# PhilippBongartz/RepeatResolver

Hardware: AMD Instinct MI355X
Metric: sum-of-pairs DP cells/sec (higher is better)
Workload: dtype u32

## Files before the change

repeatresolver_amd/csrc/pwr_device.hip:

```cpp
#include <hip/hip_runtime.h>

#include <algorithm>
#include <chrono>
#include <cstdint>
#include <cstdio>
#include <cstdlib>
#include <cstring>
#include <new>
#include <thread>
#include <type_traits>
#include <vector>

#include "pwr.h"

#define PWR_INF 0x40000000u
#define PWR_BIG 0x7fffffff

struct Hdr {
    int W;
    int nslots;
    int nfree;
    int cur;
    int status;
    int stop;
// ... 967 lines not shown
            const int rel0 = y0 + lc - a;
            int tg[C];
            int run = PWR_BIG;
#pragma unroll
            for (int i = 0; i < C; ++i) {
                const int pm1 = i ? (int)Mprev[i > 0 ? i - 1 : 0] : pm1_0;
                const int d = pm1 + ldsS[wave][cs][sxc][lc + i];
                const int u = (int)Mprev[i] + ug[i];
                accC[i] = (accC[i] << 1) | ((d <= u) ? 1u : 0u);
                const int t3 = min(min(d, u), ig[i]);
                tg[i] = ((unsigned)(rel0 + i) < (unsigned)Bx) ? t3 : PWR_BIG;
                run = min(run, tg[i]);
            }
            const int incl = wave_incl_min(run);
            const int excl = __builtin_amdgcn_update_dpp(PWR_BIG, incl, DPP_WAVE_SHR1, 0xF, 0xF, false);
            const int P_end = min(P_in, __builtin_amdgcn_readlane(incl, 63));
            int p = min(P_in, excl);
            if (x != L - 1) {
#pragma unroll
                for (int i = 0; i < C; ++i) {
                    accA[i] = (accA[i] << 1) | ((tg[i] >= p) ? 1u : 0u);
                    p = min(p, tg[i]);
                    Mprev[i] = (rel0 + i < 0) ? PWR_INF : (unsigned)(gg[i] + p);
                }
            } else {
                unsigned Mn[C];
                unsigned fa = 0;
#pragma unroll
                for (int i = 0; i < C; ++i) {
                    fa |= (tg[i] >= p) ? (1u << i) : 0u;
                    p = min(p, tg[i]);
                    Mn[i] = (rel0 + i < 0) ? PWR_INF : (unsigned)(gg[i] + p);
                }
                const unsigned mrow = needP ? ePy : PWR_INF;
                const unsigned left0 = (unsigned)__builtin_amdgcn_update_dpp((int)mrow, (int)Mn[C - 1], DPP_WAVE_SHR1, 0xF, 0xF, false);
#pragma unroll
                for (int i = 0; i < C; ++i) {
                    const unsigned lf = i ? Mn[i > 0 ? i - 1 : 0] : left0;
                    const bool inb = (unsigned)(rel0 + i) < (unsigned)Bx;
                    accA[i] = (accA[i] << 1) | ((((fa >> i) & 1u) || (inb && Mn[i] == lf)) ? 1u : 0u);
                    lastM[wave * MS + lc + i] = inb ? Mn[i] : 0xffffffffu;
                    Mprev[i] = Mn[i];
                }
            }
            nacc = (x & 15) + 1;
            if (lane == 63) {
                ST64(MBP(wave, x), P_end, x + 1);
                ST64(MBM(wave, x), Mprev[C - 1], x + 1);
                if (ms == ms_hi) ST64(PTB(x), P_end, x + 1);
            }
            ran_prev = 1;
            V2_NEXT_ROW()
        }
        if (lane == 0) __hip_atomic_store(&rdone[wave], round + 1, __ATOMIC_RELAXED, __HIP_MEMORY_SCOPE_WORKGROUP);
        __syncthreads();
        if (UNI(__hip_atomic_load(&s_done, __ATOMIC_RELAXED, __HIP_MEMORY_SCOPE_WORKGROUP)) >= NW) break;
    }
    if (round >= max_rounds) {
        if (tid == 0) { m->ok = 0; atomicCAS(&st.hdr->status, 0, PWR_ERR_INTERNAL); }
        return;
    }
    if (tid == 0) {
        m->clk = (unsigned)(__builtin_amdgcn_s_memtime() - t_clk0);
        m->rclk = (unsigned)(__builtin_amdgcn_s_memrealtime() - t_real0);
        m->rounds = round;
        atomicAdd(&st.hdr->cells_computed, m->cells);
    }
#undef MBP
#undef MBM
#undef PTB
#undef LD64
#undef LD32LO
#undef ST64
}

#ifndef PWR_INTERIOR_CLS
#define PWR_INTERIOR_CLS 0
#endif
#define V3_TICKS() ((unsigned)(__builtin_amdgcn_s_memtime() >> 10))
#define V3_TIMEOUT_TICKS (1u << 19)
#define V4_RB 128

#ifdef PWR_DIAG
#define DG_DECL unsigned long long dg_wait_fast = 0, dg_wait_gen = 0, dg_wait_setup = 0, dg_t = 0, dg_t2 = 0, dg_cyc_int = 0, dg_cyc_gen16 = 0, dg_ts1 = 0, dg_ts2 = 0, dg_tl2 = 0; unsigned dg_log = 0; unsigned dg_int = 0, dg_gen16 = 0, dg_general = 0, dg_nowork = 0, dg_runs = 0, dg_switch = 0;
#define DG_T0() dg_t = __builtin_amdgcn_s_memtime();
#define DG_ADD(ACC) ACC += __builtin_amdgcn_s_memtime() - dg_t;
#define DG_INC(CNT, N) CNT += (N);
#define DG_T2() dg_t2 = __builtin_amdgcn_s_memtime();
#define DG_ADD2(ACC) ACC += __builtin_amdgcn_s_memtime() - dg_t2;
#else
#define DG_T2()
#define DG_ADD2(ACC)
#define DG_DECL
#define DG_T0()
#define DG_ADD(ACC)
#define DG_INC(CNT, N)
#endif
template <int NW, int C, bool WG1>
__global__ __launch_bounds__(WG1 ? NW * 64 : 128) void k_fill_v3(DState st, JobBufs jb)
{
    constexpr int MS = 64 * C, RS = NW * MS;
    constexpr int NL = WG1 ? NW : 1;
    constexpr int RB = WG1 ? 64 : V4_RB;
    __shared__ __attribute__((aligned(16))) int ldsS1[NL][2][4][MS];
    __shared__ unsigned long long rP[NL][RB], rM[NL][RB];
    __shared__ int wprog[NL], wdone;
    const int vjob = WG1 ? (int)blockIdx.x : (int)(blockIdx.x + 8 * blockIdx.z), lane = threadIdx.x & 63;
    const int role = WG1 ? 0 : UNI((int)threadIdx.x >> 6);
    const int wave = WG1 ? UNI((int)threadIdx.x >> 6) : (int)blockIdx.y;
    const int lw = WG1 ? wave : 0, wr = WG1 ? (wave + 1) % NW : 0;
    if (vjob >= jb.njobs_launched * jb.smax) return;
    const int job = vjob / jb.smax;
    const SegDesc *const sd = jb.seg + (size_t)job * SEG_MAX + (vjob % jb.smax);
    JobMeta *m = &jb.meta[job];
    if (st.hdr->fallback > 0 && jb.v2_follows) return;
    if (!m->active || m->L <= 0 || !m->ok || m->wide || !sd->active || NOT_MINE(jb, job)) return;
    const int seg_xb = UNI(sd->xb), seg_fin = UNI(sd->fin);
    const int L = UNI(sd->xe) - seg_xb;
    const int Lf = seg_fin ? L - 1 : L;
    const int x_own = UNI(sd->xown) - seg_xb;
    const int g_own = x_own >> 4;
    const int chkA = x_own > 0 ? x_own : -1, chkB = seg_fin ? -1 : L;
    unsigned *const chk_w = jb.chk + (((size_t)job * (SEG_MAX + 1) + sd->s) * 2 + 0) * (size_t)jb.NC;
    unsigned *const chk_t = jb.chk + (((size_t)job * (SEG_MAX + 1) + sd->s + 1) * 2 + 1) * (size_t)jb.NC;
    const unsigned long long t_clk0 = __builtin_amdgcn_s_memtime(), t_real0 = __builtin_amdgcn_s_memrealtime();
    for (int i = threadIdx.x; i < NL * RB; i += blockDim.x) { (&rP[0][0])[i] = 0; (&rM[0][0])[i] = 0; }
    if (threadIdx.x < NL) wprog[threadIdx.x] = 0;
    if (threadIdx.x == 0) wdone = 0;
    __syncthreads();

    const int wl = (wave + NW - 1) % NW;
    const unsigned tagbase = jb.tagbase;
    const size_t gstride = (size_t)jb.gstride;
    unsigned long long *const gmy = jb.gmb + (((size_t)job * NW + wave) * gstride + (size_t)sd->grow0) * 2;
    const unsigned long long *const gleftw = jb.gmb + (((size_t)job * NW + wl) * gstride + (size_t)sd->grow0) * 2;
    const unsigned long long *const gjob = jb.gmb + ((size_t)job * NW * gstride + (size_t)sd->grow0) * 2;
#define PTOT_PTR(AP, BP, R) (gjob + (((size_t)((((AP) + (BP) - 1 - lo) / MS) % NW)) * gstride + (size_t)(R)) * 2)
    int *const abortf = &m->abort;
#define GLD(PTR) __hip_atomic_load((PTR), __ATOMIC_RELAXED, __HIP_MEMORY_SCOPE_AGENT)
#define GST(PTR, VAL, ROW) __hip_atomic_store((PTR), ((unsigned long long)(tagbase | (unsigned)((ROW) + 1)) << 32) | (unsigned)(VAL), __ATOMIC_RELAXED, __HIP_MEMORY_SCOPE_AGENT)
#define GST2(PTR, VAL, TAG) __hip_atomic_store((PTR), ((unsigned long long)(TAG) << 32) | (unsigned)(VAL), __ATOMIC_RELAXED, __HIP_MEMORY_SCOPE_AGENT)
#define TAGOF(W64) ((unsigned)((W64) >> 32))
#define LLD(REF) __hip_atomic_load(&(REF), __ATOMIC_RELAXED, __HIP_MEMORY_SCOPE_WORKGROUP)
#define LST(REF, V) __hip_atomic_store(&(REF), (V), __ATOMIC_RELAXED, __HIP_MEMORY_SCOPE_WORKGROUP)

    if (!WG1 && role == 1) {
        for (unsigned it = 0;; ++it) {
            if (UNI(LLD(wdone))) break;
            const int wx = UNI(LLD(wprog[lw]));
            const int r = wx - 1 + lane;
            const bool inr = r >= 0 && r < L;
            unsigned long long p = 0, q = 0;
            int ab = 0;
            if (inr) { p = GLD(gleftw + 2 * (size_t)r); q = GLD(gleftw + 2 * (size_t)r + 1); }
            if ((it & 15u) == 15u) ab = GLD(abortf);
            if (inr) {
                const unsigned tagr = tagbase | (unsigned)(r + 1);
                if (TAGOF(p) == tagr && TAGOF(q) == tagr) {
                    LST(rP[lw][r & (RB - 1)], p);
                    __hip_atomic_store(&rM[lw][r & (RB - 1)], q, __ATOMIC_RELEASE, __HIP_MEMORY_SCOPE_WORKGROUP);
                }
            }
            if (UNI(ab)) break;
        }
        return;
    }

    const int lo = UNI(m->lo), hi = UNI(m->hi), W = UNI(m->W), B = st.B, H = st.H;
    const int *way = jb.way + (size_t)job * jb.Lmax + seg_xb;
    const uint8_t *seq = st.seq + st.rowoff[UNI(m->k)] + seg_xb;
    const int4 *rec2 = jb.rec2 + (size_t)job * jb.colcap * 2;
    uint32_t *dirs = jb.dirs + (size_t)job * jb.dirstride + (size_t)(seg_xb >> 4) * RS;
    unsigned *lastM = jb.lastM + (size_t)job * jb.NC;
    const int lc = lane * C;
#define V4_LOADS(MSX, SLOT, AU, AG, AI, GL)                                                      \
    {                                                                                            \
        const int yq_ = lo + (MSX) * MS - 1;                                                     \
        GL = (yq_ >= lo && yq_ <= hi) ? UNI(rec2[2 * (yq_ - lo) + 1].y) : 0;                     \
        int4 p_[C];                                                                              \
        _Pragma("unroll") for (int i = 0; i < C; ++i) {                                          \
// ... 99 lines not shown
    while (x < L && !dead) {
        ran_prev = UNI(ran_prev); gacc = UNI(gacc); nacc = UNI(nacc); blk = UNI(blk); ms = UNI(ms); cs = UNI(cs); gleft = UNI(gleft);
        x = UNI(x);
#ifdef PWR_DIAG
        if (ran_prev && !dg_tl2) { dg_tl2 = __builtin_amdgcn_s_memrealtime(); if (lane == 0 && sd->s * NW + wave < 680) { tl[2] = dg_tl2; tl[5] = (unsigned long long)x; } }
#endif
        if ((ran_prev || first_pending) && x < Lf) {
            unsigned long long bOm = __builtin_amdgcn_ballot_w64((dcf & 1u) != 0);
            const bool first = UNI(first_pending) != 0;
            if (first || ((bOm >> (x & 63)) & 1ull)) {
                first_pending = 0;
                unsigned long long bPm = __builtin_amdgcn_ballot_w64((dcf & 2u) != 0);
                unsigned long long bMm = __builtin_amdgcn_ballot_w64((dcf & 4u) != 0);
                unsigned long long bTm = __builtin_amdgcn_ballot_w64((dcf & 8u) != 0);
                if (first) { bOm |= 1ull << (x & 63); bMm |= 1ull << (x & 63); }
                V4_EARLY_MASKS()
                int dcaf = (int)(dca & 0xffffffu), dcb = min(dcaf + B, W);
                unsigned dcs = min(dca >> 24, 3u) * (unsigned)(MS * 4);
                if ((x >> 4) != gacc) { V4_FLUSH() gacc = x >> 4; }
                V4_ALIGN_ACC(x & 15)
                if (lane == 0) LST(wprog[lw], x);
                unsigned mlast_v = 0;
                if (first) {
                    const unsigned tagp = tagbase | (unsigned)x;
                    const int yq = lo + ms * MS - 1;
                    const bool needM = yq >= a_prev && yq < a_prev + Bx_prev;
                    unsigned long long eT = 0, eM = 0;
                    DG_T0()
#ifdef PWR_DIAG
                    const unsigned long long ev_t0 = __builtin_amdgcn_s_memrealtime();
#endif
                    const unsigned t0 = V3_TICKS();
                    for (unsigned spin = 1;; ++spin) {
                        eT = GLD(PTOT_PTR(a_prev, Bx_prev, x - 1));
                        eM = LLD(rM[lw][(x - 1) & (RB - 1)]);
                        if (UNI(TAGOF(eT)) == tagp && (!needM || UNI(TAGOF(eM)) == tagp)) break;
                        if ((spin & 1023u) == 0 && (V3_TICKS() - t0 > V3_TIMEOUT_TICKS || UNI(GLD(abortf)))) { dead = true; break; }
                        __builtin_amdgcn_s_sleep(1);
                    }
                    DG_ADD(dg_wait_gen)
#ifdef PWR_DIAG
                    if (lane == 0 && dg_general < 36) {
                        unsigned long long *ev = jb.diag + ((size_t)job * 32 + wave) * 4096 + 16 + 3 * dg_general;
                        ev[0] = (unsigned long long)x; ev[1] = ev_t0; ev[2] = __builtin_amdgcn_s_memrealtime();
                    }
#endif
                    DG_INC(dg_general, 1)
                    if (dead) break;
                    const int eTx = (int)UNI((unsigned)eT);
#pragma unroll
                    for (int i = 0; i < C; ++i) Mprev[i] = (unsigned)eTx;
                    mlast_v = yq < a_prev ? PWR_INF - (unsigned)gleft : (needM ? UNI((unsigned)eM) : (unsigned)eTx);
                    ran_prev = 1;
                } else if ((bMm >> (x & 63)) & 1ull) {
                    const unsigned tagp = tagbase | (unsigned)x;
                    unsigned long long w_ = LLD(rM[lw][(x - 1) & (RB - 1)]);
                    if (UNI(TAGOF(w_)) != tagp) {
                        DG_T0()
                        const unsigned t0 = V3_TICKS();
                        for (unsigned spin = 1;; ++spin) {
                            w_ = LLD(rM[lw][(x - 1) & (RB - 1)]);
                            if (UNI(TAGOF(w_)) == tagp) break;
                            if ((spin & 1023u) == 0 && (V3_TICKS() - t0 > V3_TIMEOUT_TICKS || UNI(GLD(abortf)))) { dead = true; break; }
                            __builtin_amdgcn_s_sleep(1);
                        }
                        DG_ADD(dg_wait_setup)
                        if (dead) break;
                    }
                    mlast_v = (unsigned)w_;
                }
                int ycol[C];
#pragma unroll
                for (int i = 0; i < C; ++i) ycol[i] = lo + ms * MS + lc + i;
                const char *const stab = (const char *)&ldsS1[lw][cs][0][lc];
                int sgr[C];
                {
                    const int *const srow0 = (const int *)(stab + __builtin_amdgcn_readlane((int)dcs, x & 63));
#pragma unroll
                    for (int i = 0; i < C; ++i) sgr[i] = srow0[i];
                }
                int af_done = a_prev;
                int g_af = 0, g_be = 0, g_cs = 0, g_cp = -1;
                DG_INC(dg_runs, 1)
                while (true) {
                    const int r_beg = x & 15, g0 = x - r_beg, r0 = g0 & 63;
                    int nrun = __builtin_ctz(~((unsigned)(bOm >> (r0 + r_beg)) & 0xffffu) | (1u << (16 - r_beg)));
                    nrun = min(nrun, Lf - x);
                    if (nrun <= 0) break;
                    const unsigned nPm = (unsigned)(bPm >> r0) & 0xffffu, kMm = (unsigned)(bMm >> r0) & 0xffffu, eTm = (unsigned)(bTm >> r0) & 0xffffu;
                    const unsigned p0 = (nPm >> r_beg) & 1u, m0 = (kMm >> r_beg) & 1u, t0_ = (eTm >> r_beg) & 1u;
                    const unsigned diff = ((nPm ^ (0u - p0)) | (kMm ^ (0u - m0)) | ((p0 & m0) ? 0u : (eTm ^ (0u - t0_)))) & 0xffffu;
                    const int nsame = __builtin_ctz((diff >> r_beg) | 0x10000u);
                    const bool mixed16 = r_beg == 0 && nrun == 16 && nsame < 16;
                    const int r_e = mixed16 ? 16 : r_beg + min(nrun, nsame);
                    const unsigned et_here = (eTm >> r_beg) & ((1u << (r_e - r_beg)) - 1u);
                    const int cls = mixed16 ? 3 : ((p0 & m0) ? (et_here ? 1 : 0) : ((p0 | m0 | t0_) == 0u ? 2 : 3));
                    if (gacc < 0) gacc = x >> 4;
#ifdef PWR_DIAG
                    if (!dg_ts1 && x >= 1024) dg_ts1 = __builtin_amdgcn_s_memrealtime();
                    if (!dg_ts2 && x >= 2048) dg_ts2 = __builtin_amdgcn_s_memrealtime();
#endif
                    if (WG1) {
                        const int need = g0 + 16 - RB + 2;
                        if (need > 0 && UNI(LLD(wprog[wr])) < need) {
                            DG_T0()
                            const unsigned t0 = V3_TICKS();
                            for (unsigned spin = 1;; ++spin) {
                                if (UNI(LLD(wprog[wr])) >= need) break;
                                if ((spin & 1023u) == 0 && (V3_TICKS() - t0 > V3_TIMEOUT_TICKS || UNI(GLD(abortf)))) { dead = true; break; }
                                __builtin_amdgcn_s_sleep(1);
                            }
                            DG_ADD(dg_wait_setup)
                            if (dead) break;
                        }
                    }
                    unsigned long long *const gq0 = gmy + 2 * (size_t)g0;
                    const unsigned tag_g0 = tagbase | (unsigned)g0;
                    const unsigned long long *const ringM = &rM[lw][g0 & (RB - 1)], *const ringP = &rP[lw][g0 & (RB - 1)];
                    if (g0 != g_cp) {
                        const int src = 4 * min(r0 + lane, 63);
                        g_af = __builtin_amdgcn_ds_bpermute(src, dcaf);
                        g_be = __builtin_amdgcn_ds_bpermute(src, dcb);
                        g_cs = __builtin_amdgcn_ds_bpermute(src, (int)dcs);
                        g_cp = g0;
                    }
                    auto group_row = [&](const int r, auto cls_, auto bits_) __attribute__((always_inline)) {
                        constexpr int CLS = decltype(cls_)::value;
                        constexpr bool BITS = decltype(bits_)::value;
                        bool bP = CLS <= 1 || CLS == 4, bM = CLS <= 1 || CLS == 4;
                        if (CLS == 3) { bP = (nPm >> r) & 1u; bM = (kMm >> r) & 1u; }
                        int af = 0, bend = 0;
                        if (CLS >= 2) af = __builtin_amdgcn_readlane(g_af, r);
                        if (CLS == 1 || CLS == 3 || CLS == 4) bend = __builtin_amdgcn_readlane(g_be, r);
                        const int Mleft_v = bM ? (int)mlast_v : (int)PWR_INF - gleft;
                        const int pm1_0 = __builtin_amdgcn_update_dpp(Mleft_v, (int)Mprev[C - 1], DPP_WAVE_SHR1, 0xF, 0xF, false);
                        int tg[C];
                        int run = FBIG;
#pragma unroll
                        for (int i = 0; i < C; ++i) {
                            const int pm1 = i ? (int)Mprev[i > 0 ? i - 1 : 0] : pm1_0;
                            const int d = pm1 + sgr[i];
                            const int u = (int)Mprev[i] + ug[i];
                            if (BITS) accC[i] = acc_push(accC[i], __builtin_amdgcn_sicmp(d, u, ICMP_SLE));
                            const int t3 = min(min(d, u), ig[i]);
                            bool inb = true;
                            if (CLS == 1 || CLS == 4) inb = ycol[i] < bend;
                            if (CLS == 2) inb = ycol[i] >= af;
                            if (CLS == 3) inb = (unsigned)(ycol[i] - af) < (unsigned)(bend - af);
                            tg[i] = inb ? t3 : FBIG;
                            run = min(run, tg[i]);
                        }
                        unsigned long long fM = 0;
                        unsigned fP = 0;
                        if (CLS != 2) {
                            fM = LLD(ringM[r]);
                            __builtin_amdgcn_sched_barrier(0);
                            fP = __hip_atomic_load((const unsigned *)&ringP[r], __ATOMIC_RELAXED, __HIP_MEMORY_SCOPE_WORKGROUP);
                        }
                        __builtin_amdgcn_sched_barrier(0);
#define V4_SCAN_STEP(CTRL, RMASK) { const int t_ = __builtin_amdgcn_update_dpp(PWR_BIG, incl, CTRL, RMASK, 0xF, false); incl = min(incl, t_); }
#define V4_FENCE() __builtin_amdgcn_sched_barrier(0)
                        int incl = run;
                        V4_SCAN_STEP(DPP_ROW_SHR(1), 0xF) V4_FENCE();
                        const int soff = __builtin_amdgcn_readlane(g_cs, r + 1);
                        V4_FENCE(); V4_SCAN_STEP(DPP_ROW_SHR(2), 0xF) V4_FENCE();
                        const int *const srow = (const int *)(stab + soff);
                        V4_FENCE(); V4_SCAN_STEP(DPP_ROW_SHR(4), 0xF) V4_FENCE();
#pragma unroll
                        for (int i = 0; i < C; ++i) sgr[i] = srow[i];
                        V4_FENCE(); V4_SCAN_STEP(DPP_ROW_SHR(8), 0xF) V4_FENCE();
                        const unsigned tagx = tag_g0 + (unsigned)(r + 1);
                        V4_FENCE(); V4_SCAN_STEP(DPP_ROW_BCAST15, 0xA) V4_FENCE();
                        V4_FENCE(); V4_SCAN_STEP(DPP_ROW_BCAST31, 0xC) V4_FENCE();
#undef V4_SCAN_STEP
#undef V4_FENCE
                        if (bP && __builtin_expect(UNI(TAGOF(fM)) != tagx, 0)) {
                            DG_T0()
                            const unsigned t0 = V3_TICKS();
                            for (unsigned spin = 1; !dead; ++spin) {
                                fM = LLD(ringM[r]);
                                __builtin_amdgcn_sched_barrier(0);
                                fP = __hip_atomic_load((const unsigned *)&ringP[r], __ATOMIC_RELAXED, __HIP_MEMORY_SCOPE_WORKGROUP);
                                if (UNI(TAGOF(fM)) == tagx) break;
                                if ((spin & 1023u) == 0 && (V3_TICKS() - t0 > V3_TIMEOUT_TICKS || UNI(GLD(abortf)))) { dead = true; break; }
                                __builtin_amdgcn_s_sleep(1);
                            }
                            DG_ADD(dg_wait_fast)
                        }
                        const int P_in_v = bP ? (int)fP : PWR_BIG;
                        const int P_end_v = min(P_in_v, incl);
                        const int pq = min(P_in_v, FBIG);
                        int p = min(__builtin_amdgcn_update_dpp(pq, incl, DPP_WAVE_SHR1, 0xF, 0xF, false), pq);
#pragma unroll
                        for (int i = 0; i < C; ++i) {
                            if (BITS) accA[i] = acc_push(accA[i], __builtin_amdgcn_sicmp(tg[i], p, ICMP_SGE));
                            p = min(p, tg[i]);
                            Mprev[i] = (unsigned)(CLS == 0 ? p : min(p, ig[i]));
                        }
                        mlast_v = (unsigned)fM;
                        if (lane == 63) {
                            if (WG1) {
                                GST2(gq0 + 2 * r, P_end_v, tagx);
                                LST(rP[wr][(g0 + r) & (RB - 1)], ((unsigned long long)tagx << 32) | (unsigned)P_end_v);
                                LST(rM[wr][(g0 + r) & (RB - 1)], ((unsigned long long)tagx << 32) | (unsigned)Mprev[C - 1]);
                            } else {
                                typedef unsigned v4u_ __attribute__((ext_vector_type(4)));
                                v4u_ w4_; w4_.x = (unsigned)P_end_v; w4_.y = tagx; w4_.z = Mprev[C - 1]; w4_.w = tagx;
                                asm volatile("global_store_dwordx4 %0, %1, %2 sc1\n\ts_nop 1" :: "v"(16 * r), "v"(w4_), "s"(gq0) : "memory");
                            }
                        }
                    };
                    int r_end = r_e;
                    DG_T2()
                    using WithBits = std::integral_constant<bool, true>;
                    using NoBits = std::integral_constant<bool, false>;
                    const bool warmup = (x >> 4) < g_own;
                    if (warmup && r_beg == 0 && r_e == 16 && cls != 3) {
                        if (cls == 0) {
#pragma unroll
                            for (int r = 0; r < 16; ++r) group_row(r, std::integral_constant<int, PWR_INTERIOR_CLS>{}, NoBits{});
                            DG_INC(dg_int, 16)
                            DG_ADD2(dg_cyc_int)
                        } else if (cls == 1) {
#pragma unroll
                            for (int r = 0; r < 16; ++r) group_row(r, std::integral_constant<int, 1>{}, NoBits{});
                        } else {
#pragma unroll
                            for (int r = 0; r < 16; ++r) group_row(r, std::integral_constant<int, 2>{}, NoBits{});
                        }
                    } else if (cls == 0 && r_beg == 0 && r_e == 16) {
#pragma unroll
                        for (int r = 0; r < 16; ++r) group_row(r, std::integral_constant<int, PWR_INTERIOR_CLS>{}, WithBits{});
                        DG_INC(dg_int, 16)
                        DG_ADD2(dg_cyc_int)
                    } else if (cls == 1 && r_beg == 0 && r_e == 16) {
#pragma unroll
                        for (int r = 0; r < 16; ++r) group_row(r, std::integral_constant<int, 1>{}, WithBits{});
                    } else if (cls == 3 && r_beg == 0 && r_e == 16) {
#pragma unroll
                        for (int r = 0; r < 16; ++r) group_row(r, std::integral_constant<int, 3>{}, WithBits{});
                    } else if (cls == 2 && r_beg == 0 && r_e == 16) {
#pragma unroll
                        for (int r = 0; r < 16; ++r) group_row(r, std::integral_constant<int, 2>{}, WithBits{});
                    } else {
                        int r = r_beg;
                        for (; r < r_end && (r & 3) && !dead; ++r) group_row(r, std::integral_constant<int, 3>{}, WithBits{});
#define V4_BLOCKS(K) for (; r + 4 <= r_end && !dead; r += 4) { group_row(r, std::integral_constant<int, K>{}, WithBits{}); group_row(r + 1, std::integral_constant<int, K>{}, WithBits{}); \
                                                               group_row(r + 2, std::integral_constant<int, K>{}, WithBits{}); group_row(r + 3, std::integral_constant<int, K>{}, WithBits{}); }
                        if (cls == 0) V4_BLOCKS(0)
                        else if (cls == 1) V4_BLOCKS(1)
                        else if (cls == 2) V4_BLOCKS(2)
#undef V4_BLOCKS
                        for (; r < r_end && !dead; ++r) group_row(r, std::integral_constant<int, 3>{}, WithBits{});
                        r_end = r;
                    }
                    if (!(cls == 0 && r_beg == 0 && r_e == 16)) { DG_INC(dg_gen16, r_end - r_beg) DG_ADD2(dg_cyc_gen16) }
                    x = g0 + r_end;
#ifdef PWR_DIAG
                    if (lane == 0 && dg_log < 1270) {
                        unsigned long long *lg = jb.diag + ((size_t)job * 32 + wave) * 4096 + 256 + 3 * dg_log;
                        lg[0] = (unsigned long long)x | ((unsigned long long)cls << 32) | ((unsigned long long)(r_end - r_beg) << 40); lg[1] = __builtin_amdgcn_s_memrealtime();
                        lg[2] = dg_wait_fast + dg_wait_gen + dg_wait_setup;
                    }
                    dg_log += 1;
#endif
                    af_done = __builtin_amdgcn_readlane(dcaf, (x - 1) & 63);
                    if ((x & 15) == 0) {
                        uint32_t *d_ = dirs + (size_t)gacc * RS + (size_t)wave * MS + (size_t)lc;
#pragma unroll
                        for (int i = 0; i < C; ++i) { if (gacc >= g_own) d_[i] = accA[i] | (accC[i] << 16); accA[i] = accC[i] = 0; }
                        gacc = -1; nacc = 0;
                        V4_CHK_STORE(x, af_done, min(af_done + B, W))
                    } else nacc = x & 15;
                    if (dead || x >= Lf) break;
                    if ((x >> 6) != blk) {
                        V4_ROTATE_BLOCK()
                        bOm = __builtin_amdgcn_ballot_w64((dcf & 1u) != 0); bPm = __builtin_amdgcn_ballot_w64((dcf & 2u) != 0);
                        bMm = __builtin_amdgcn_ballot_w64((dcf & 4u) != 0); bTm = __builtin_amdgcn_ballot_w64((dcf & 8u) != 0);
                        V4_EARLY_MASKS()
                        dcaf = (int)(dca & 0xffffffu); dcb = min(dcaf + B, W);
                        dcs = min(dca >> 24, 3u) * (unsigned)(MS * 4);
                        g_cp = -1;
                        const int *const srow0 = (const int *)(stab + __builtin_amdgcn_readlane((int)dcs, 0));
#pragma unroll
                        for (int i = 0; i < C; ++i) sgr[i] = srow0[i];
                    }
                    if (lane == 0) LST(wprog[lw], x);
                }
                a_prev = af_done; Bx_prev = min(B, W - af_done);
                if (dead) break;
                if (x < L) {
                    if ((x >> 6) != blk) V4_ROTATE_BLOCK()
                    a = max(0, __builtin_amdgcn_readlane(wcur, x & 63) - H);
                    sx = __builtin_amdgcn_readlane(scur, x & 63);
                }
                if (lane == 0) LST(wprog[lw], x);
                continue;
            }
        }
        if (dead || x >= L) break;

        x = UNI(x); ms = UNI(ms); msn = UNI(msn); a = UNI(a); a_prev = UNI(a_prev); Bx_prev = UNI(Bx_prev);
        sx = UNI(sx); gacc = UNI(gacc); nacc = UNI(nacc); blk = UNI(blk); gleft = UNI(gleft); gleftn = UNI(gleftn); ran_prev = UNI(ran_prev); cs = UNI(cs);
        const int Bx = min(B, W - a);
        const int ms_lo = (a - lo) / MS, ms_hi = (a + Bx - 1 - lo) / MS;
        if (ms < ms_lo) {
            ms += NW;
            if (ms == msn) {
#pragma unroll
                for (int i = 0; i < C; ++i) { ug[i] = nu[i]; gg[i] = ng[i]; ig[i] = ni[i]; }
                gleft = gleftn;
                cs ^= 1;
            } else {
                while (ms < ms_lo) ms += NW;
                V4_LOADS(ms, cs, ug, gg, ig, gleft)
            }
            DG_INC(dg_switch, 1)
            msn = ms + NW;
            V4_LOADS(msn, cs ^ 1, nu, ng, ni, gleftn)
            ran_prev = 0;
            continue;
        }
        if (ms > ms_hi) {
            const int y0s = lo + ms * MS;
            const int anf_l = (int)(dca & 0xffffffu);
            const unsigned long long wm = __builtin_amdgcn_ballot_w64(min(anf_l + B, W) > y0s) >> (x & 63);
            const int xn = min(wm ? x + __builtin_ctzll(wm) : ((x >> 6) + 1) << 6, L);
            int xs = xn;
            if (wm && xn < Lf) {
                const int anf_up = __builtin_amdgcn_update_dpp(0x3fffffff, anf_l, DPP_WAVE_SHR1, 0xF, 0xF, false);
                const unsigned long long tears = __builtin_amdgcn_ballot_w64(anf_l >= min(anf_up + B, W)) >> (x & 63);
                const unsigned long long tm = tears & (~0ull >> (63 - (xn - x))) & ~1ull;
                xs = max(x, xn & ~15);
                if (tm) xs = max(xs, x + 63 - __builtin_clzll(tm));
                if (xs < 1) xs = xn;
                const int an = __builtin_amdgcn_readlane(anf_l, xn & 63);
                if (ms < (an - lo) / MS) { xs = xn; first_pending = 0; }
                else { early_lo = xs; early_hi = xn; first_pending = xs > 0 ? 1 : 0; }
            }
            DG_INC(dg_nowork, xs - x)
            if (xs > x) {
                const int al = __builtin_amdgcn_readlane((int)dca, (xs - 1) & 63) & 0xffffff;
                a_prev = al; Bx_prev = min(B, W - al);
            }
// ... 48 lines not shown
            DG_ADD(dg_wait_gen)
            DG_INC(dg_general, 1)
            if (dead) break;
        }
        int Mleft = (int)PWR_INF;
        if (x == 0) Mleft = (src_c < 0 || yq == src_c) ? -gleft : (int)PWR_INF - gleft;
        else if (yq < a_prev) Mleft = (int)PWR_INF - gleft;
        else if (needM) Mleft = (int)eMy;
        else Mleft = (int)eTx;
        const int P_in = needP ? (int)ePx : PWR_BIG;
        if (x > 0 && !ran_prev) {
#pragma unroll
            for (int i = 0; i < C; ++i) Mprev[i] = eTx;
        }
        if ((x >> 4) != gacc) { V4_FLUSH() gacc = x >> 4; }
        V4_ALIGN_ACC(x & 15)
        const int pm1_0 = __builtin_amdgcn_update_dpp(Mleft, (int)Mprev[C - 1], DPP_WAVE_SHR1, 0xF, 0xF, false);
        const int sxc = min(max(sx, 0), 3);
        const int rel0 = y0 + lc - a;
        int tg[C];
        int run = PWR_BIG;
#pragma unroll
        for (int i = 0; i < C; ++i) {
            const int pm1 = i ? (int)Mprev[i > 0 ? i - 1 : 0] : pm1_0;
            const int d = pm1 + ldsS1[lw][cs][sxc][lc + i];
            const int u = (int)Mprev[i] + ug[i];
            accC[i] = (accC[i] << 1) | ((d <= u) ? 1u : 0u);
            const int t3 = min(min(d, u), ig[i]);
            tg[i] = ((unsigned)(rel0 + i) < (unsigned)Bx) ? t3 : PWR_BIG;
            run = min(run, tg[i]);
        }
        const int incl = wave_incl_min(run);
        const int excl = __builtin_amdgcn_update_dpp(PWR_BIG, incl, DPP_WAVE_SHR1, 0xF, 0xF, false);
        const int P_end = min(P_in, __builtin_amdgcn_readlane(incl, 63));
        int p = min(P_in, excl);
        if (x != Lf) {
#pragma unroll
            for (int i = 0; i < C; ++i) {
                accA[i] = (accA[i] << 1) | ((tg[i] >= p) ? 1u : 0u);
                p = min(p, tg[i]);
                Mprev[i] = (unsigned)((rel0 + i < 0) ? ig[i] : p);
            }
        } else {
            unsigned Mn[C];
            unsigned fa = 0;
#pragma unroll
            for (int i = 0; i < C; ++i) {
                fa |= (tg[i] >= p) ? (1u << i) : 0u;
                p = min(p, tg[i]);
                Mn[i] = (rel0 + i < 0) ? PWR_INF : (unsigned)(gg[i] + p);
                Mprev[i] = (unsigned)((rel0 + i < 0) ? ig[i] : p);
            }
            const unsigned mrow = needP ? (unsigned)gleft + ePy : PWR_INF;
            const unsigned left0 = (unsigned)__builtin_amdgcn_update_dpp((int)mrow, (int)Mn[C - 1], DPP_WAVE_SHR1, 0xF, 0xF, false);
#pragma unroll
            for (int i = 0; i < C; ++i) {
                const unsigned lf = i ? Mn[i > 0 ? i - 1 : 0] : left0;
                const bool inb = (unsigned)(rel0 + i) < (unsigned)Bx;
                accA[i] = (accA[i] << 1) | ((((fa >> i) & 1u) || (inb && Mn[i] == lf)) ? 1u : 0u);
                lastM[wave * MS + lc + i] = inb ? Mn[i] : 0xffffffffu;
            }
        }
        nacc = (x & 15) + 1;
        if (lane == 63) {
            GST(gmy + 2 * (size_t)x, P_end, x);
            if (WG1) {
                const unsigned long long tg_ = (unsigned long long)(tagbase | (unsigned)(x + 1)) << 32;
                LST(rP[wr][x & (RB - 1)], tg_ | (unsigned)P_end);
                LST(rM[wr][x & (RB - 1)], tg_ | (unsigned)Mprev[C - 1]);
            } else GST(gmy + 2 * (size_t)x + 1, Mprev[C - 1], x);
        }
        ran_prev = 1;
        V4_CHK_STORE(x + 1, a, a + Bx)
        V4_NEXT_ROW()
    }
    V4_FLUSH()
#ifdef PWR_DIAG
    if (lane == 0) {
        unsigned long long *dgp = jb.diag + ((size_t)job * 32 + wave) * 4096;
        dgp[0] = __builtin_amdgcn_s_memtime() - t_clk0; dgp[1] = dg_wait_fast; dgp[2] = dg_wait_gen; dgp[3] = dg_wait_setup;
        dgp[4] = ((unsigned long long)dg_int << 32) | dg_gen16; dgp[5] = ((unsigned long long)dg_general << 32) | dg_nowork;
        dgp[6] = ((unsigned long long)dg_runs << 32) | dg_switch; dgp[7] = (unsigned long long)L;
        dgp[12] = dg_log; dgp[8] = dg_cyc_gen16; dgp[9] = dg_ts1; dgp[10] = dg_ts2; dgp[11] = dg_cyc_int;
    }
#endif
#ifdef PWR_DIAG
    if (lane == 0 && sd->s * NW + wave < 680) { tl[3] = __builtin_amdgcn_s_memrealtime(); tl[4] = (unsigned long long)L | ((unsigned long long)(dg_wait_fast + dg_wait_gen + dg_wait_setup) << 20); }
#endif
    if (lane == 0) { LST(wprog[lw], 0x7fffffff); LST(wdone, 1); }
    if (dead) {
        if (lane == 0) __hip_atomic_store(abortf, 1, __ATOMIC_RELAXED, __HIP_MEMORY_SCOPE_AGENT);
        return;
    }
    if (wave == 0 && lane == 0) {
        if (sd->s == 0) {
            m->clk = (unsigned)(__builtin_amdgcn_s_memtime() - t_clk0);
            m->rclk = (unsigned)(__builtin_amdgcn_s_memrealtime() - t_real0);
            m->rounds = 0;
        }
        atomicAdd(&st.hdr->cells_computed, sd->cells);
    }
#undef V4_CHK_STORE
#undef V4_EARLY_MASKS
#undef PTOT_PTR
#undef GLD
#undef GST
#undef GST2
#undef TAGOF
#undef LLD
#undef LST
#undef V4_LOADS
#undef V4_ALIGN_ACC
#undef V4_FLUSH
#undef V4_ROTATE_BLOCK
#undef V4_NEXT_ROW
}

__device__ __forceinline__ bool seg_check_applies(const DState &st, const JobBufs &jb, int job, const JobMeta *m)
{
    return m->active && m->L > 0 && m->ok && !m->wide && !m->abort && !(st.hdr->fallback > 0 && jb.v2_follows) && !NOT_MINE(jb, job) && m->nseg > 1;
}

__device__ __forceinline__ void seg_check_body(const DState &st, const JobBufs &jb, const int job, const int s, const int tid)
{
    __shared__ int s_min[4], s_max[4], s_bad;
    JobMeta *m = &jb.meta[job];
    if (!seg_check_applies(st, jb, job, m)) return;
    if (s >= m->nseg) return;
    const SegDesc *sd = jb.seg + (size_t)job * SEG_MAX + s;
    const int xr = sd->xown - 1;
    const int lo = m->lo, W = m->W, B = st.B, H = st.H, RS = jb.NC;
    const int a = max(0, jb.way[(size_t)job * jb.Lmax + xr] - H), Bx = min(B, W - a);
    unsigned *cw = jb.chk + (((size_t)job * (SEG_MAX + 1) + s) * 2 + 0) * (size_t)jb.NC;
    unsigned *ct = jb.chk + (((size_t)job * (SEG_MAX + 1) + s) * 2 + 1) * (size_t)jb.NC;
    if (tid == 0) s_bad = 0;
    __syncthreads();
    int dmin = INT_MAX, dmax = INT_MIN, bad = 0;
    for (int j = tid; j < Bx; j += 256) {
        const int idx = (a + j - lo) % RS;
        const unsigned vw = cw[idx], vt = ct[idx];
        if (vw == 0xffffffffu || vt == 0xffffffffu) bad = 1;
        else if ((vw >= PWR_INF) != (vt >= PWR_INF)) bad = 1;
        else if (vw < PWR_INF) { const int d = (int)(vw - vt); dmin = min(dmin, d); dmax = max(dmax, d); }
    }
    for (int o = 32; o > 0; o >>= 1) { dmin = min(dmin, __shfl_xor(dmin, o)); dmax = max(dmax, __shfl_xor(dmax, o)); }
    if ((tid & 63) == 0) { s_min[tid >> 6] = dmin; s_max[tid >> 6] = dmax; }
    if (bad) s_bad = 1;
    __syncthreads();
    for (int j = tid; j < RS; j += 256) { cw[j] = 0xffffffffu; ct[j] = 0xffffffffu; }
    if (tid == 0) {
        const int lo_ = min(min(s_min[0], s_min[1]), min(s_min[2], s_min[3])), hi_ = max(max(s_max[0], s_max[1]), max(s_max[2], s_max[3]));
        if (s_bad || (lo_ != INT_MAX && lo_ != hi_)) __hip_atomic_store(&m->segfail, 1, __ATOMIC_RELAXED, __HIP_MEMORY_SCOPE_AGENT);
        if (s == 1) { atomicAdd(&st.hdr->seg_jobs, 1ull); atomicAdd(&st.hdr->segs, (unsigned long long)m->nseg); }
        __hip_atomic_fetch_add(&jb.chkdone[job], 1, __ATOMIC_RELEASE, __HIP_MEMORY_SCOPE_AGENT);
    }
}

__global__ __launch_bounds__(256) void k_seg_check(DState st, JobBufs jb)
{
    seg_check_body(st, jb, (int)blockIdx.x, (int)blockIdx.y + 1, (int)threadIdx.x);
}

#define F64_NT 1024
#define F64_INF (1ll << 62)
__global__ __launch_bounds__(F64_NT) void k_fill64(DState st, JobBufs jb)
{
// ... 2771 lines not shown
    return PWR_OK;
}

extern "C" int pwr_reset_stats(pwr_ctx *c)
{
    if (!c) return PWR_ERR_ARG;
    if (c->on_device) {
        if (hipSetDevice(c->device) != hipSuccess) return PWR_ERR_DEVICE;
        int rc0 = drain_events(c);
        if (rc0) return rc0;
    }
    c->stats = pwr_stats{};
    if (c->on_device) {
        if (hipSetDevice(c->device) != hipSuccess) return PWR_ERR_DEVICE;
        HIPC(hipStreamSynchronize(c->stream));
        HIPC(hipMemset(&c->st.hdr->cells_computed, 0, 16 * sizeof(unsigned long long)));
        HIPC(hipMemset(&c->st.hdr->rows_jumped, 0, sizeof(unsigned long long)));
    }
    return PWR_OK;
}

extern "C" int pwr_debug_last_job(pwr_ctx *c, int *L, int *entry, int *W, int *way, int *newcol, int cap)
{
    if (!c || !c->on_device) return PWR_ERR_ARG;
    if (hipSetDevice(c->device) != hipSuccess) return PWR_ERR_DEVICE;
    HIPC(hipStreamSynchronize(c->stream));
    JobMeta m;
    HIPC(hipMemcpy(&m, c->jb.meta, sizeof m, hipMemcpyDeviceToHost));
    if (L) *L = m.L;
    if (entry) *entry = m.entry;
    if (W) *W = m.W;
    const int n = std::min(cap, m.L);
    if (way && n > 0) HIPC(hipMemcpy(way, c->jb.way, sizeof(int) * n, hipMemcpyDeviceToHost));
    if (newcol && n > 0) HIPC(hipMemcpy(newcol, c->jb.newcol, sizeof(int) * n, hipMemcpyDeviceToHost));
    return PWR_OK;
}

extern "C" int pwr_debug_row_columns(pwr_ctx *c, int k, int *out, int cap)
{
    if (!c || !c->on_device || k < 0 || k >= c->T || !out) return PWR_ERR_ARG;
    if (hipSetDevice(c->device) != hipSuccess) return PWR_ERR_DEVICE;
    const int L = c->rowlen[k];
    if (L == 0) return 0;
    int *d = nullptr;
    int rc = dmalloc(c, &d, (size_t)L);
    if (rc) return rc;
    hipLaunchKernelGGL(k_rowcols, dim3(32), dim3(256), 0, c->stream, c->st, k, d);
    std::vector<int> h(L);
    if (hipMemcpyAsync(h.data(), d, sizeof(int) * L, hipMemcpyDeviceToHost, c->stream) != hipSuccess || hipStreamSynchronize(c->stream) != hipSuccess) { dfree(c, d); return PWR_ERR_DEVICE; }
    dfree(c, d);
    memcpy(out, h.data(), sizeof(int) * std::min(L, cap));
    return L;
}

extern "C" int pwr_debug_rounds(pwr_ctx *c)
{
    if (!c || !c->on_device) return PWR_ERR_ARG;
    if (hipSetDevice(c->device) != hipSuccess) return PWR_ERR_DEVICE;
    if (hipStreamSynchronize(c->stream) != hipSuccess) return PWR_ERR_DEVICE;
    JobMeta m;
    if (hipMemcpy(&m, c->jb.meta, sizeof m, hipMemcpyDeviceToHost) != hipSuccess) return PWR_ERR_DEVICE;
    return m.rounds;
}

extern "C" int pwr_debug_phase_times(pwr_ctx *c, unsigned long long *out)
{
    if (!c || !c->on_device || !out) return PWR_ERR_ARG;
    if (hipSetDevice(c->device) != hipSuccess) return PWR_ERR_DEVICE;
    HIPC(hipStreamSynchronize(c->stream));
    HIPC(hipMemcpy(out, c->st.hdr->dbg, sizeof(unsigned long long) * 32, hipMemcpyDeviceToHost));
    HIPC(hipMemset(c->st.hdr->dbg, 0, sizeof(unsigned long long) * 32));
    return PWR_OK;
}

extern "C" int pwr_debug_fill_diag(pwr_ctx *c, unsigned long long *out)
{
    if (!c || !c->on_device || !out) return PWR_ERR_ARG;
    if (hipSetDevice(c->device) != hipSuccess) return PWR_ERR_DEVICE;
    HIPC(hipStreamSynchronize(c->stream));
    HIPC(hipMemcpy(out, c->jb.diag, sizeof(unsigned long long) * 32 * 4096, hipMemcpyDeviceToHost));
    return PWR_OK;
}

extern "C" int pwr_debug_fill_clock(pwr_ctx *c, double *mhz, double *fill_us)
{
    if (!c || !c->on_device) return PWR_ERR_ARG;
    if (hipSetDevice(c->device) != hipSuccess) return PWR_ERR_DEVICE;
    HIPC(hipStreamSynchronize(c->stream));
    JobMeta m;
    HIPC(hipMemcpy(&m, c->jb.meta, sizeof m, hipMemcpyDeviceToHost));
    if (mhz) *mhz = m.rclk ? 100.0 * (double)m.clk / (double)m.rclk : 0.0;
    if (fill_us) *fill_us = (double)m.rclk / 100.0;
    return PWR_OK;
}
```

Before: 54.95 billion.

## Merge consecutive same-class 16-row groups into multi-group runs

```diff
diff --git a/repeatresolver_amd/csrc/pwr_device.hip b/repeatresolver_amd/csrc/pwr_device.hip
--- a/repeatresolver_amd/csrc/pwr_device.hip
+++ b/repeatresolver_amd/csrc/pwr_device.hip
@@ -1073,20 +1073,73 @@
 #define V4_RB 128
 
 #ifdef PWR_DIAG
-#define DG_DECL unsigned long long dg_wait_fast = 0, dg_wait_gen = 0, dg_wait_setup = 0, dg_t = 0, dg_t2 = 0, dg_cyc_int = 0, dg_cyc_gen16 = 0, dg_ts1 = 0, dg_ts2 = 0, dg_tl2 = 0; unsigned dg_log = 0; unsigned dg_int = 0, dg_gen16 = 0, dg_general = 0, dg_nowork = 0, dg_runs = 0, dg_switch = 0;
+#define DG_DECL unsigned long long dg_wait_fast = 0, dg_wait_gen = 0, dg_wait_setup = 0, dg_t = 0, dg_t2 = 0, dg_cyc_int = 0, dg_cyc_gen16 = 0, dg_ts1 = 0, dg_ts2 = 0, dg_tl2 = 0; unsigned dg_log = 0; unsigned dg_int = 0, dg_gen16 = 0, dg_general = 0, dg_nowork = 0, dg_runs = 0, dg_switch = 0; \
+    unsigned long long dg_tg = 0, dg_glue = 0; unsigned dg_ngl = 0, dg_gcont = 0, dg_gother = 0; int dg_pkey = -1, dg_pend = -1;
 #define DG_T0() dg_t = __builtin_amdgcn_s_memtime();
 #define DG_ADD(ACC) ACC += __builtin_amdgcn_s_memtime() - dg_t;
 #define DG_INC(CNT, N) CNT += (N);
 #define DG_T2() dg_t2 = __builtin_amdgcn_s_memtime();
 #define DG_ADD2(ACC) ACC += __builtin_amdgcn_s_memtime() - dg_t2;
+#define DG_GLUE_RESET() dg_tg = 0;
+#define DG_GROUP_BEGIN(KEY, G0, WHOLE)                                                           \
+    {                                                                                            \
+        if (dg_tg) { dg_glue += __builtin_amdgcn_s_memtime() - dg_tg; dg_ngl += 1; }             \
+        if ((WHOLE) && dg_pkey == (int)(KEY) && dg_pend == (G0)) dg_gcont += 1; else dg_gother += 1;  \
+        dg_pkey = (WHOLE) ? (int)(KEY) : -1; dg_pend = (G0) + 16;                                \
+    }
+#define DG_GROUP_END() dg_tg = __builtin_amdgcn_s_memtime();
 #else
 #define DG_T2()
 #define DG_ADD2(ACC)
+#define DG_GLUE_RESET()
+#define DG_GROUP_BEGIN(KEY, G0, WHOLE)
+#define DG_GROUP_END()
 #define DG_DECL
 #define DG_T0()
 #define DG_ADD(ACC)
 #define DG_INC(CNT, N)
 #endif
+struct V4Run { int cls, r_e, ngrp; };
+__host__ __device__ static inline int v4_group_cls(const unsigned nPm, const unsigned kMm, const unsigned eTm)
+{
+    const unsigned p0 = nPm & 1u, m0 = kMm & 1u, t0_ = eTm & 1u;
+    const unsigned diff = ((nPm ^ (0u - p0)) | (kMm ^ (0u - m0)) | ((p0 & m0) ? 0u : (eTm ^ (0u - t0_)))) & 0xffffu;
+    if (diff) return 3;
+    return (p0 & m0) ? (eTm ? 1 : 0) : ((p0 | m0 | t0_) == 0u ? 2 : 3);
+}
+__host__ __device__ static inline V4Run v4_classify_run(const unsigned long long bOm, const unsigned long long bPm, const unsigned long long bMm,
+                                                        const unsigned long long bTm, const int x, const int g_own, const int Lf,
+                                                        const int early_lo, const int early_hi)
+{
+    V4Run out = {3, x & 15, 0};
+    const int r_beg = x & 15, g0 = x - r_beg, r0 = g0 & 63;
+    int nrun = __builtin_ctz(~((unsigned)(bOm >> (r0 + r_beg)) & 0xffffu) | (1u << (16 - r_beg)));
+    nrun = nrun < Lf - x ? nrun : Lf - x;
+    if (nrun <= 0) return out;
+    const unsigned nPm = (unsigned)(bPm >> r0) & 0xffffu, kMm = (unsigned)(bMm >> r0) & 0xffffu, eTm = (unsigned)(bTm >> r0) & 0xffffu;
+    out.ngrp = 1;
+    if (r_beg == 0 && nrun == 16) {
+        out.cls = v4_group_cls(nPm, kMm, eTm);
+        out.r_e = 16;
+        const bool warm = (g0 >> 4) < g_own;
+        if (early_hi >= g0 && early_lo < g0 + 16) return out;
+        for (int k = 1; r0 + 16 * k < 64; ++k) {
+            const int gk = g0 + 16 * k, rk = r0 + 16 * k;
+            if (gk + 16 > Lf || ((gk >> 4) < g_own) != warm || (early_hi >= gk && early_lo < gk + 16)) break;
+            if (((unsigned)(bOm >> rk) & 0xffffu) != 0xffffu) break;
+            if (v4_group_cls((unsigned)(bPm >> rk) & 0xffffu, (unsigned)(bMm >> rk) & 0xffffu, (unsigned)(bTm >> rk) & 0xffffu) != out.cls) break;
+            out.ngrp = k + 1;
+        }
+        return out;
+    }
+    const unsigned p0 = (nPm >> r_beg) & 1u, m0 = (kMm >> r_beg) & 1u, t0_ = (eTm >> r_beg) & 1u;
+    const unsigned diff = ((nPm ^ (0u - p0)) | (kMm ^ (0u - m0)) | ((p0 & m0) ? 0u : (eTm ^ (0u - t0_)))) & 0xffffu;
+    const int nsame = __builtin_ctz((diff >> r_beg) | 0x10000u);
+    out.r_e = r_beg + (nrun < nsame ? nrun : nsame);
+    const unsigned et_here = (eTm >> r_beg) & ((1u << (out.r_e - r_beg)) - 1u);
+    out.cls = (p0 & m0) ? (et_here ? 1 : 0) : ((p0 | m0 | t0_) == 0u ? 2 : 3);
+    return out;
+}
 template <int NW, int C, bool WG1>
 __global__ __launch_bounds__(WG1 ? NW * 64 : 128) void k_fill_v3(DState st, JobBufs jb)
 {
@@ -1352,19 +1405,17 @@
                 int af_done = a_prev;
                 int g_af = 0, g_be = 0, g_cs = 0, g_cp = -1;
                 DG_INC(dg_runs, 1)
+                DG_GLUE_RESET()
                 while (true) {
-                    const int r_beg = x & 15, g0 = x - r_beg, r0 = g0 & 63;
-                    int nrun = __builtin_ctz(~((unsigned)(bOm >> (r0 + r_beg)) & 0xffffu) | (1u << (16 - r_beg)));
-                    nrun = min(nrun, Lf - x);
-                    if (nrun <= 0) break;
-                    const unsigned nPm = (unsigned)(bPm >> r0) & 0xffffu, kMm = (unsigned)(bMm >> r0) & 0xffffu, eTm = (unsigned)(bTm >> r0) & 0xffffu;
-                    const unsigned p0 = (nPm >> r_beg) & 1u, m0 = (kMm >> r_beg) & 1u, t0_ = (eTm >> r_beg) & 1u;
-                    const unsigned diff = ((nPm ^ (0u - p0)) | (kMm ^ (0u - m0)) | ((p0 & m0) ? 0u : (eTm ^ (0u - t0_)))) & 0xffffu;
-                    const int nsame = __builtin_ctz((diff >> r_beg) | 0x10000u);
-                    const bool mixed16 = r_beg == 0 && nrun == 16 && nsame < 16;
-                    const int r_e = mixed16 ? 16 : r_beg + min(nrun, nsame);
-                    const unsigned et_here = (eTm >> r_beg) & ((1u << (r_e - r_beg)) - 1u);
-                    const int cls = mixed16 ? 3 : ((p0 & m0) ? (et_here ? 1 : 0) : ((p0 | m0 | t0_) == 0u ? 2 : 3));
+                    const int r_beg = x & 15;
+                    int g0 = x - r_beg, r0 = g0 & 63;
+                    const V4Run run = v4_classify_run(bOm, bPm, bMm, bTm, x, g_own, Lf, early_lo, early_hi);
+                    if (run.ngrp <= 0) break;
+                    unsigned nPm = (unsigned)(bPm >> r0) & 0xffffu, kMm = (unsigned)(bMm >> r0) & 0xffffu;
+                    const int r_e = run.r_e, cls = run.cls;
+#ifdef PWR_DIAG
+                    const int dg_x0 = x;
+#endif
                     if (gacc < 0) gacc = x >> 4;
 #ifdef PWR_DIAG
                     if (!dg_ts1 && x >= 1024) dg_ts1 = __builtin_amdgcn_s_memrealtime();
@@ -1384,9 +1435,9 @@
                             if (dead) break;
                         }
                     }
-                    unsigned long long *const gq0 = gmy + 2 * (size_t)g0;
-                    const unsigned tag_g0 = tagbase | (unsigned)g0;
-                    const unsigned long long *const ringM = &rM[lw][g0 & (RB - 1)], *const ringP = &rP[lw][g0 & (RB - 1)];
+                    unsigned long long *gq0 = gmy + 2 * (size_t)g0;
+                    unsigned tag_g0 = tagbase | (unsigned)g0;
+                    const unsigned long long *ringM = &rM[lw][g0 & (RB - 1)], *ringP = &rP[lw][g0 & (RB - 1)];
                     if (g0 != g_cp) {
                         const int src = 4 * min(r0 + lane, 63);
                         g_af = __builtin_amdgcn_ds_bpermute(src, dcaf);
@@ -1481,38 +1532,73 @@
                         }
                     };
                     int r_end = r_e;
-                    DG_T2()
                     using WithBits = std::integral_constant<bool, true>;
                     using NoBits = std::integral_constant<bool, false>;
                     const bool warmup = (x >> 4) < g_own;
+#define V4_RUN_NEXT(NAF, NBE, NCS)                                                               \
+                    {                                                                            \
+                        const int xg_ = g0 + 16;                                                 \
+                        if (xg_ == chkA || xg_ == chkB) break;        \
+                        uint32_t *d_ = dirs + (size_t)gacc * RS + (size_t)wave * MS + (size_t)lc; \
+                        _Pragma("unroll") for (int i = 0; i < C; ++i) { if (gacc >= g_own) d_[i] = accA[i] | (accC[i] << 16); accA[i] = accC[i] = 0; } \
+                        if (lane == 0) LST(wprog[lw], xg_);                                      \
+                        if (WG1) {                                                               \
+                            const int need_ = xg_ + 16 - RB + 2;                                 \
+                            if (need_ > 0 && UNI(LLD(wprog[wr])) < need_) {                      \
+                                DG_T0()                                                          \
+                                const unsigned t0_ = V3_TICKS();                                 \
+                                for (unsigned spin = 1;; ++spin) {                               \
+                                    if (UNI(LLD(wprog[wr])) >= need_) break;                     \
+                                    if ((spin & 1023u) == 0 && (V3_TICKS() - t0_ > V3_TIMEOUT_TICKS || UNI(GLD(abortf)))) { dead = true; break; } \
+                                    __builtin_amdgcn_s_sleep(1);                                 \
+                                }                                                                \
+                                DG_ADD(dg_wait_setup)                                            \
+                                if (dead) break;      \
+                            }                                                                    \
+                        }                                                                        \
+                        gacc += 1; g0 = xg_; r0 += 16;                                           \
+                        gq0 += 32; tag_g0 += 16u; ringM += 16; ringP += 16;                      \
+                        nPm = (unsigned)(bPm >> r0) & 0xffffu; kMm = (unsigned)(bMm >> r0) & 0xffffu; \
+                        g_af = NAF; g_be = NBE; g_cs = NCS; g_cp = g0;                           \
+                    }
+#ifdef PWR_DIAG
+#define V4_RUN_DIAG_BEGIN() { if (!dg_ts1 && g0 >= 1024) dg_ts1 = __builtin_amdgcn_s_memrealtime(); if (!dg_ts2 && g0 >= 2048) dg_ts2 = __builtin_amdgcn_s_memrealtime(); } \
+                        DG_GROUP_BEGIN(cls | (warmup ? 8 : 0) | ((g0 >> 6) << 4), g0, true) DG_T2()
+#define V4_RUN_DIAG_END() if (cls == 0) { DG_INC(dg_int, 16) DG_ADD2(dg_cyc_int) } else { DG_INC(dg_gen16, 16) DG_ADD2(dg_cyc_gen16) } DG_GROUP_END()
+#else
+#define V4_RUN_DIAG_BEGIN()
+#define V4_RUN_DIAG_END()
+#endif
+#define V4_RUN(CLSK, BITS)                                                                       \
+                    for (int gi = run.ngrp;; --gi) {                                             \
+                        int n_af = 0, n_be = 0, n_cs = 0;                                        \
+                        if (gi > 1) {                                                            \
+                            const int src_ = 4 * min(r0 + 16 + lane, 63);                        \
+                            n_af = __builtin_amdgcn_ds_bpermute(src_, dcaf);                     \
+                            n_be = __builtin_amdgcn_ds_bpermute(src_, dcb);                      \
+                            n_cs = __builtin_amdgcn_ds_bpermute(src_, (int)dcs);                 \
+                        }                                                                        \
+                        V4_RUN_DIAG_BEGIN()                                                      \
+                        _Pragma("unroll") for (int r = 0; r < 16; ++r) group_row(r, std::integral_constant<int, CLSK>{}, BITS{}); \
+                        V4_RUN_DIAG_END()                                                        \
+                        if (gi <= 1 || dead) break;                                              \
+                        V4_RUN_NEXT(n_af, n_be, n_cs)                                            \
+                    }
                     if (warmup && r_beg == 0 && r_e == 16 && cls != 3) {
-                        if (cls == 0) {
-#pragma unroll
-                            for (int r = 0; r < 16; ++r) group_row(r, std::integral_constant<int, PWR_INTERIOR_CLS>{}, NoBits{});
-                            DG_INC(dg_int, 16)
-                            DG_ADD2(dg_cyc_int)
-                        } else if (cls == 1) {
-#pragma unroll
-                            for (int r = 0; r < 16; ++r) group_row(r, std::integral_constant<int, 1>{}, NoBits{});
-                        } else {
-#pragma unroll
-                            for (int r = 0; r < 16; ++r) group_row(r, std::integral_constant<int, 2>{}, NoBits{});
-                        }
+                        if (cls == 0) { V4_RUN(PWR_INTERIOR_CLS, NoBits) }
+                        else if (cls == 1) { V4_RUN(1, NoBits) }
+                        else { V4_RUN(2, NoBits) }
                     } else if (cls == 0 && r_beg == 0 && r_e == 16) {
-#pragma unroll
-                        for (int r = 0; r < 16; ++r) group_row(r, std::integral_constant<int, PWR_INTERIOR_CLS>{}, WithBits{});
-                        DG_INC(dg_int, 16)
-                        DG_ADD2(dg_cyc_int)
+                        V4_RUN(PWR_INTERIOR_CLS, WithBits)
                     } else if (cls == 1 && r_beg == 0 && r_e == 16) {
-#pragma unroll
-                        for (int r = 0; r < 16; ++r) group_row(r, std::integral_constant<int, 1>{}, WithBits{});
+                        V4_RUN(1, WithBits)
                     } else if (cls == 3 && r_beg == 0 && r_e == 16) {
-#pragma unroll
-                        for (int r = 0; r < 16; ++r) group_row(r, std::integral_constant<int, 3>{}, WithBits{});
+                        V4_RUN(3, WithBits)
                     } else if (cls == 2 && r_beg == 0 && r_e == 16) {
-#pragma unroll
-                        for (int r = 0; r < 16; ++r) group_row(r, std::integral_constant<int, 2>{}, WithBits{});
+                        V4_RUN(2, WithBits)
                     } else {
+                        DG_GROUP_BEGIN(-1, g0, false)
+                        DG_T2()
                         int r = r_beg;
                         for (; r < r_end && (r & 3) && !dead; ++r) group_row(r, std::integral_constant<int, 3>{}, WithBits{});
 #define V4_BLOCKS(K) for (; r + 4 <= r_end && !dead; r += 4) { group_row(r, std::integral_constant<int, K>{}, WithBits{}); group_row(r + 1, std::integral_constant<int, K>{}, WithBits{}); \
@@ -1523,13 +1609,18 @@
 #undef V4_BLOCKS
                         for (; r < r_end && !dead; ++r) group_row(r, std::integral_constant<int, 3>{}, WithBits{});
                         r_end = r;
+                        DG_INC(dg_gen16, r_end - r_beg) DG_ADD2(dg_cyc_gen16)
+                        DG_GROUP_END()
                     }
-                    if (!(cls == 0 && r_beg == 0 && r_e == 16)) { DG_INC(dg_gen16, r_end - r_beg) DG_ADD2(dg_cyc_gen16) }
+#undef V4_RUN
+#undef V4_RUN_NEXT
+#undef V4_RUN_DIAG_BEGIN
+#undef V4_RUN_DIAG_END
                     x = g0 + r_end;
 #ifdef PWR_DIAG
                     if (lane == 0 && dg_log < 1270) {
                         unsigned long long *lg = jb.diag + ((size_t)job * 32 + wave) * 4096 + 256 + 3 * dg_log;
-                        lg[0] = (unsigned long long)x | ((unsigned long long)cls << 32) | ((unsigned long long)(r_end - r_beg) << 40); lg[1] = __builtin_amdgcn_s_memrealtime();
+                        lg[0] = (unsigned long long)x | ((unsigned long long)cls << 32) | ((unsigned long long)(x - dg_x0) << 40); lg[1] = __builtin_amdgcn_s_memrealtime();
                         lg[2] = dg_wait_fast + dg_wait_gen + dg_wait_setup;
                     }
                     dg_log += 1;
@@ -1744,6 +1835,12 @@
         dgp[4] = ((unsigned long long)dg_int << 32) | dg_gen16; dgp[5] = ((unsigned long long)dg_general << 32) | dg_nowork;
         dgp[6] = ((unsigned long long)dg_runs << 32) | dg_switch; dgp[7] = (unsigned long long)L;
         dgp[12] = dg_log; dgp[8] = dg_cyc_gen16; dgp[9] = dg_ts1; dgp[10] = dg_ts2; dgp[11] = dg_cyc_int;
+        dgp[13] = dg_glue; dgp[14] = ((unsigned long long)dg_ngl << 32) | dg_gcont; dgp[15] = dg_gother;
+        if (sd->s * NW + wave < 680) {
+            unsigned long long *gs = jb.diag + ((size_t)job * 32 + 30) * 4096 + (size_t)(sd->s * NW + wave) * 6;
+            gs[0] = dgp[0]; gs[1] = dg_glue; gs[2] = dgp[14]; gs[3] = dg_gother; gs[4] = dg_wait_fast + dg_wait_gen + dg_wait_setup;
+            gs[5] = (unsigned long long)L | ((unsigned long long)tagbase << 32);
+        }
     }
 #endif
 #ifdef PWR_DIAG
@@ -4681,6 +4778,14 @@
     return PWR_OK;
 }
 
+extern "C" int pwr_debug_fill_group_run(const unsigned long long *masks, int x, int g_own, int Lf, int early_lo, int early_hi, int *out)
+{
+    if (!masks || !out || x < 0) return PWR_ERR_ARG;
+    const V4Run r = v4_classify_run(masks[0], masks[1], masks[2], masks[3], x, g_own, Lf, early_lo, early_hi);
+    out[0] = r.cls; out[1] = r.r_e; out[2] = r.ngrp;
+    return PWR_OK;
+}
+
 extern "C" int pwr_debug_fill_clock(pwr_ctx *c, double *mhz, double *fill_us)
 {
     if (!c || !c->on_device) return PWR_ERR_ARG;
```

After: 55.13 billion (median of 6 runs). About the same (+0.3%).
